# patflick/psac

Hardware: AMD Instinct MI355X
Metric: MChars/s SA+LCP build; rank-pair radix-sort HBM GB/s vs peak (higher is better)
Workload: dtype u64

## Files before the change

### include/psacx.h

```cpp
#ifndef PSACX_H
#define PSACX_H

#include <stddef.h>
#include <stdint.h>

#ifdef __cplusplus
extern "C" {
#endif

typedef struct psacx_ctx psacx_ctx;

enum {
    PSACX_OK = 0,
    PSACX_EINVAL = -1,
    PSACX_ERANGE = -2,
    PSACX_ENOMEM = -3,
    PSACX_EHIP = -4,
    PSACX_EDEVICE = -5,
    PSACX_ENOGPU = -6
};

enum {
    PSACX_LCP = 1u,
    PSACX_NO_FAST = 2u,
// ... 13 lines not shown

typedef struct psacx_stats {
    uint32_t sigma;
    uint32_t bits_per_char;
    uint32_t k;
    uint32_t n_rounds;
    psacx_round rounds[PSACX_MAX_ROUNDS];
    double ms_total;
    double ms_alphabet, ms_kmer, ms_sort_hist, ms_sort_scatter, ms_rebucket, ms_isa_scatter,
           ms_gather, ms_compact, ms_rmq_build, ms_finalize;
    double ms_sort_scatter3, ms_sort_tilehist, ms_sort_scatter2;
    uint64_t scatter_launches[3];
    uint64_t scatter_records[3];
    uint64_t scatter_bytes[3];
    uint64_t hist_bytes;
    uint64_t workspace_bytes;
    uint64_t onew_passes;
    uint64_t heavy_rounds;
    uint64_t heavy_records;
    uint64_t light_records;
    uint64_t level_gathers;
    double ms_host[9];
    uint64_t locate_fetches[2];
} psacx_stats;


#define PSACX_STREAM_DEFAULT ((void*)(intptr_t)-1)
int psacx_create(psacx_ctx** out, int device, void* stream);
void psacx_destroy(psacx_ctx* ctx);
const char* psacx_strerror(int code);
const char* psacx_last_hip_error(const psacx_ctx* ctx);
int psacx_trim(psacx_ctx* ctx);

enum {
    PSACX_OPT_RESET = 0, PSACX_OPT_FORCE_DIET, PSACX_OPT_DIET_CAP, PSACX_OPT_ONE_STAGE, PSACX_OPT_TIES_RADIX, PSACX_OPT_NO_ONE_WORD,
    PSACX_OPT_ONE_WORD_ALWAYS, PSACX_OPT_ONE_WORD_MIN, PSACX_OPT_WIDEN_LAST, PSACX_OPT_NO_DIGIT_BYTES, PSACX_OPT_NO_BUCKET_SORT,
    PSACX_OPT_ISA_UPDATE, PSACX_OPT_GATHER, PSACX_OPT_NO_HEAVY, PSACX_OPT_NO_WHOLE, PSACX_OPT_NO_LAZY_RANKS, PSACX_OPT_NO_EARLY_OUT,
    PSACX_OPT_NO_SPREAD_CURSORS, PSACX_OPT_LOCATE_SHAPE, PSACX_OPT_LOCATE_COUNT, PSACX_OPT_COUNT
};
int psacx_configure(psacx_ctx* ctx, int option, uint64_t value);
int psacx_configure_from_env(psacx_ctx* ctx);
const char* psacx_debug_env(const char* name);

int psacx_construct_u32(psacx_ctx* ctx, const uint8_t* text, uint64_t n, uint32_t k,
                        uint32_t flags, uint32_t* SA, uint32_t* ISA, uint32_t* LCP);
int psacx_construct_u64(psacx_ctx* ctx, const uint8_t* text, uint64_t n, uint32_t k,
                        uint32_t flags, uint64_t* SA, uint64_t* ISA, uint64_t* LCP);
int psacx_construct_dev_u32(psacx_ctx* ctx, const uint8_t* d_text, uint64_t n, uint32_t k,
                            uint32_t flags, uint32_t* d_SA, uint32_t* d_ISA, uint32_t* d_LCP);
int psacx_construct_dev_u64(psacx_ctx* ctx, const uint8_t* d_text, uint64_t n, uint32_t k,
                            uint32_t flags, uint64_t* d_SA, uint64_t* d_ISA, uint64_t* d_LCP);

int psacx_construct_lc_u32(psacx_ctx* ctx, const uint8_t* text, uint64_t n, uint32_t k, uint32_t flags,
                           uint32_t* SA, uint32_t* ISA, uint32_t* LCP, uint8_t* Lc);
int psacx_construct_lc_u64(psacx_ctx* ctx, const uint8_t* text, uint64_t n, uint32_t k, uint32_t flags,
                           uint64_t* SA, uint64_t* ISA, uint64_t* LCP, uint8_t* Lc);
int psacx_construct_lc_dev_u32(psacx_ctx* ctx, const uint8_t* d_text, uint64_t n, uint32_t k, uint32_t flags,
                               uint32_t* d_SA, uint32_t* d_ISA, uint32_t* d_LCP, uint8_t* d_Lc);
int psacx_construct_lc_dev_u64(psacx_ctx* ctx, const uint8_t* d_text, uint64_t n, uint32_t k, uint32_t flags,
                               uint64_t* d_SA, uint64_t* d_ISA, uint64_t* d_LCP, uint8_t* d_Lc);

// ... 178 lines not shown
```

### psac_amd/_lib.py

```python
import ctypes as C
import os

_HERE = os.path.dirname(os.path.abspath(__file__))
LIB_PATH = os.path.join(_HERE, "lib", "libpsacx.so")

PSACX_LCP = 1
PSACX_NO_FAST = 2
PSACX_PROFILE = 4
PSACX_MAX_ROUNDS = 72

OPTIONS = {"reset": 0, "force_diet": 1, "diet_cap": 2, "one_stage": 3, "ties_radix": 4, "no_one_word": 5, "one_word_always": 6, "one_word_min": 7,
           "widen_last": 8, "no_digit_bytes": 9, "no_bucket_sort": 10, "isa_update": 11, "gather": 12, "no_heavy": 13, "no_whole": 14, "no_lazy_ranks": 15, "no_early_out": 16,
           "no_spread_cursors": 17, "locate_shape": 18, "locate_count": 19}
MULTI_OPTIONS = {"layout": 1, "slab": 2, "output_slack": 3, "trace": 4, "wire_piece": 5, "pieces": 6, "check_chunks": 7, "global_refine_sort": 8,
                 "one_stage": 9, "two_word": 10, "one_word": 11, "no_slices": 12, "slice_wide": 13, "slice_shape": 14}
MULTI_FORCE_WIRE, MULTI_NO_RCCL, MULTI_SHM = 1, 2, 4
ENV_KNOBS = bool(os.environ.get("PSACX_ENV_KNOBS"))
if ENV_KNOBS and os.environ.get("PSACX_LIB"):
    LIB_PATH = os.environ["PSACX_LIB"]

EXPORTS = [
    "psacx_create", "psacx_destroy", "psacx_strerror", "psacx_last_hip_error", "psacx_trim", "psacx_configure", "psacx_configure_from_env", "psacx_debug_env",
    "psacx_construct_u32", "psacx_construct_u64", "psacx_construct_dev_u32", "psacx_construct_dev_u64",
    "psacx_construct_gsa_u32", "psacx_construct_gsa_u64", "psacx_construct_gsa_dev_u32", "psacx_construct_gsa_dev_u64",
    "psacx_construct_lc_u32", "psacx_construct_lc_u64", "psacx_construct_lc_dev_u32", "psacx_construct_lc_dev_u64",
    "psacx_get_stats", "psacx_profile", "psacx_check_dev_u32", "psacx_check_dev_u64", "psacx_check_gsa_dev_u32", "psacx_check_gsa_dev_u64", "psacx_pair_sort_dev_u32", "psacx_pair_sort_dev_u64", "psacx_ansv_u32",
    "psacx_ansv_u64", "psacx_ansv_dev_u32", "psacx_ansv_dev_u64", "psacx_suffix_tree_u32", "psacx_suffix_tree_u64", "psacx_suffix_tree_dev_u32", "psacx_suffix_tree_dev_u64",
    "psacx_check_suffix_tree_dev_u32", "psacx_check_suffix_tree_dev_u64",
    "psacx_suffix_tree_gsa_u32", "psacx_suffix_tree_gsa_u64", "psacx_suffix_tree_gsa_dev_u32", "psacx_suffix_tree_gsa_dev_u64",
    "psacx_check_suffix_tree_gsa_dev_u32", "psacx_check_suffix_tree_gsa_dev_u64", "psacx_dev_alloc", "psacx_dev_free", "psacx_copy_h2d", "psacx_copy_d2h", "psacx_sync",
    "psacx_rand_dna", "psacx_synth_text_dev",
    "psacx_lookup_table_dev_u32", "psacx_lookup_table_dev_u64", "psacx_locate_dev_u32", "psacx_locate_dev_u64", "psacx_locate_u32", "psacx_locate_u64",
    "psacx_multi_create", "psacx_multi_unique_id", "psacx_multi_create_rank", "psacx_multi_destroy", "psacx_multi_nranks",
    "psacx_multi_nlocal", "psacx_multi_uses_rccl", "psacx_multi_last_error", "psacx_multi_ctx", "psacx_multi_construct_dev_u32",
    "psacx_multi_construct_dev_u64", "psacx_multi_construct_u32", "psacx_multi_construct_u64", "psacx_multi_get_stats",
    "psacx_multi_check_dev_u32", "psacx_multi_check_dev_u64", "psacx_multi_check_gsa_dev_u32", "psacx_multi_check_gsa_dev_u64", "psacx_multi_ansv_dev_u32", "psacx_multi_ansv_dev_u64",
# ... 1 lines not shown
    "psacx_multi_suffix_tree_dev_u32", "psacx_multi_suffix_tree_dev_u64", "psacx_multi_suffix_tree_u32", "psacx_multi_suffix_tree_u64",
    "psacx_multi_left_chars_dev_u32", "psacx_multi_left_chars_dev_u64", "psacx_multi_construct_lc_u32", "psacx_multi_construct_lc_u64",
    "psacx_multi_configure", "psacx_multi_configure_from_env", "psacx_multi_create_ex", "psacx_multi_create_rank_ex", "psacx_multi_get_memory", "psacx_multi_transport", "psacx_multi_get_wire", "psacx_multi_get_phases", "psacx_multi_last_form",
]


class Round(C.Structure):
    _fields_ = [("h", C.c_uint64), ("active", C.c_uint64), ("unfinished_buckets", C.c_uint64),
                ("unfinished_elements", C.c_uint64), ("sort_passes", C.c_uint32),
                ("sort_passes_skipped", C.c_uint32)]


class Stats(C.Structure):
    _fields_ = [("sigma", C.c_uint32), ("bits_per_char", C.c_uint32), ("k", C.c_uint32),
                ("n_rounds", C.c_uint32), ("rounds", Round * PSACX_MAX_ROUNDS),
                ("ms_total", C.c_double), ("ms_alphabet", C.c_double), ("ms_kmer", C.c_double),
                ("ms_sort_hist", C.c_double), ("ms_sort_scatter", C.c_double), ("ms_rebucket", C.c_double),
                ("ms_isa_scatter", C.c_double), ("ms_gather", C.c_double), ("ms_compact", C.c_double),
                ("ms_rmq_build", C.c_double), ("ms_finalize", C.c_double),
                ("ms_sort_scatter3", C.c_double), ("ms_sort_tilehist", C.c_double), ("ms_sort_scatter2", C.c_double),
                ("scatter_launches", C.c_uint64 * 3), ("scatter_records", C.c_uint64 * 3),
                ("scatter_bytes", C.c_uint64 * 3), ("hist_bytes", C.c_uint64), ("workspace_bytes", C.c_uint64), ("onew_passes", C.c_uint64),
                ("heavy_rounds", C.c_uint64), ("heavy_records", C.c_uint64), ("light_records", C.c_uint64), ("level_gathers", C.c_uint64),
                ("ms_host", C.c_double * 9), ("locate_fetches", C.c_uint64 * 2)]


class PsacxError(RuntimeError):
    def __init__(self, code, msg):
        RuntimeError.__init__(self, "psacx error %d: %s" % (code, msg))
        self.code = code


_lib = None


def load():
    global _lib
    if _lib is not None:
        return _lib
    if not os.path.exists(LIB_PATH):
        raise ImportError("libpsacx.so not built (%s); run `python -c 'import __graft_entry__ as g; g.build()'`"
                          % LIB_PATH)
    try:
        import torch
    except ImportError:
        pass
    lib = C.CDLL(LIB_PATH, mode=C.RTLD_GLOBAL)
# ... 111 lines not shown
```

### psac_amd/csrc/construct.hpp

```cpp
#pragma once
#include <chrono>
#include <thread>
#include "engine.hpp"
#include "bucket_sort.hpp"
#include "heavy_keys.hpp"

namespace psacx {

constexpr int SCAN_ITEMS = 8;
#ifndef RB1W_BLOCK
#define RB1W_BLOCK 512
#endif
template <typename T> struct ScanCfg {
    static constexpr int BLOCK = sizeof(T) == 8 ? 512 : 768;
    static constexpr int TILE = BLOCK * SCAN_ITEMS;
};
constexpr int SCAN_TILE_MIN = 512 * SCAN_ITEMS;

constexpr unsigned SCAN_CHUNKS = 4096, SCAN_CHUNK = 1024 * 4;
template <typename T> struct Work {
    T *bsa;
    SortBufs<T> x, y;
    SortBufs<T> ry;
    T *pos_a, *pos_b;
// ... 291 lines not shown
        kin = o.k1; vin = o.k2;
    }
    const uint64_t nwin = (n + (1ull << INV_WINDOW_BITS) - 1) >> INV_WINDOW_BITS;
    hipLaunchKernelGGL((window_scatter_kernel<T, T, 512>), dim3((unsigned)nwin), dim3(512), 0, c->stream, kin, vin, n, d_isa);
    PSACX_HIP(c, hipGetLastError());
    return PSACX_OK;
}

template <typename T> struct IsaLevels {
    static constexpr int PB = 512, PI = 16, WB = ISA_NARROW_WB, CB = ISA_NARROW_CB;
    psacx_ctx* c; unsigned* cursors; uint64_t n; int lv9; uint64_t* lvl_a; bool open; unsigned stripes;
    unsigned* c0() const { return cursors; }
    unsigned* c1() const { return cursors + 1024; }
    int begin(psacx_ctx* ctx, unsigned* d_cursors, uint64_t n_, uint64_t* a, const Knobs& kn) {
        c = ctx; cursors = d_cursors; n = n_; lvl_a = a; open = true;
        lv9 = isa_narrow_levels<T>(n, kn);
        stripes = isa_stripes(kn);
        if (lv9 < 1 || lv9 > 2) { c->hip_err = "ISA update by levels: text size out of range"; return PSACX_EINVAL; }
        PSACX_HIP(c, hipMemsetAsync(cursors, 0, (1024 + (size_t)(n >> WB) + 1) * sizeof(unsigned), c->stream));
        return PSACX_OK;
    }
    int add(const uint64_t* pairs, uint64_t cnt, const ulonglong2* skip = nullptr) {
        static_assert((PB * PI) % ScanCfg<T>::TILE == 0 || sizeof(T) != 8, "a tile of pairs covers whole scan tiles");
        hipLaunchKernelGGL((partition_packed_kernel<T, PB, PI, 0, CB>), dim3(striped_grid((cnt + PB * PI - 1) / (PB * PI), stripes)), dim3(PB), 0, c->stream, (const T*)nullptr,
                           (const T*)nullptr, pairs, lvl_a, cnt, isa_narrow_shift(lv9, 0), lv9 == 1 ? c1() : c0(), (uint64_t)0, (const unsigned*)nullptr, 0u,
                           (const uint32_t*)nullptr, (uint64_t)0, (uint64_t)0, skip, skip ? (unsigned)((PB * PI) / ScanCfg<T>::TILE) : 0u, stripes);
        PSACX_HIP(c, hipGetLastError());
        return PSACX_OK;
    }
    int finish(T* d_isa, uint64_t* lvl_b) {
        open = false;
        const uint64_t* last = lvl_a;
        if (lv9 == 2) {
            hipLaunchKernelGGL((partition_packed_kernel<T, PB, PI, 0, CB>), dim3(striped_grid((n + PB * PI - 1) / (PB * PI), stripes)), dim3(PB), 0, c->stream, (const T*)nullptr,
                               (const T*)nullptr, (const uint64_t*)lvl_a, lvl_b, n, (unsigned)WB, c1(), (uint64_t)0, (const unsigned*)c0(), isa_narrow_shift(lv9, 0),
                               (const uint32_t*)nullptr, (uint64_t)0, (uint64_t)0, (const ulonglong2*)nullptr, 0u, stripes);
            PSACX_HIP(c, hipGetLastError());
            last = lvl_b;
        }
        hipLaunchKernelGGL((window_store_sparse_kernel<T, 1024, WB>), dim3((unsigned)((n + (1ull << WB) - 1) >> WB)), dim3(1024), 0, c->stream, last, (const unsigned*)c1(), n, d_isa);
        PSACX_HIP(c, hipGetLastError());
        return PSACX_OK;
    }
};

template <typename T>
// ... 383 lines not shown
        T* const pyr1 = (WITH_LCP && w.pyr.nlev > 1) ? w.pyr.lvl[1] : (T*)nullptr;
        isa_hist_ready = !fuse32 && isa_radix_levels<T>(n, kn) && (uint64_t)ScanCfg<T>::TILE == (uint64_t)ScatterCfg<T>::TILE;
        unsigned* const sa_hist = isa_hist_ready ? reinterpret_cast<unsigned*>(w.sc.d_desc + 256) : (unsigned*)nullptr;
        if (gsa) {
            PSACX_TRY((run_carries<T, false, true>(c, w, sorted.k1, sorted.k2, nullptr, n, d_sa, ks)));
            hipLaunchKernelGGL((rebucket_first_kernel<T, ScanCfg<T>::BLOCK, SCAN_ITEMS, WITH_LCP, true>), dim3((unsigned)ntiles),
                               dim3(ScanCfg<T>::BLOCK), 0, c->stream, sorted.k1, sorted.k2, d_sa, n, ks, w.bsa, d_lcp,
                               w.d_carry, w.d_nact, w.d_nunf, n, Boundary<T>(), pyr1, sa_hist, (int)INV_WINDOW_BITS);
        } else if (fuse32) {
            PSACX_TRY((run_carries<T, false>(c, w, sorted.k1, sorted.k2, nullptr, n, d_sa, ks)));
            PSACX_HIP(c, hipMemsetAsync(w.d_cursors, 0, ((size_t)1 << ISA_NARROW_CB) * sizeof(unsigned) + sizeof(unsigned), c->stream));
            launch_rebucket_first_fused<T, WITH_LCP>(c, (unsigned)ntiles, sorted.k1, sorted.k2, d_sa, n, ks, w.bsa, d_lcp, w.d_carry, w.d_nact,
                                                     w.d_nunf, pyr1, reinterpret_cast<uint32_t*>(w.x.v), reinterpret_cast<uint32_t*>(w.y.v),
                                                     isa_narrow_shift(isa_levels32(n), 0), w.d_cursors);
        } else if (fuse_l1 && onew_recs) {
            if constexpr (sizeof(T) == 8) {
                hipLaunchKernelGGL(last_head_1w_kernel<0>, dim3((unsigned)((ntiles + 3) / 4)), dim3(256), 0, c->stream, reinterpret_cast<const uint64_t*>(sorted.k1),
                                   reinterpret_cast<const uint64_t*>(onew_w1), reinterpret_cast<const uint64_t*>(sorted.k2), n, (unsigned)ScanCfg<T>::TILE, ntiles,
                                   w.d_carry, ks, onew_view);
                PSACX_HIP(c, hipGetLastError());
                PSACX_TRY(scan_carries<T>(c, w, ntiles));
                PSACX_HIP(c, hipMemsetAsync(w.d_cursors, 0, ((size_t)1 << ISA_NARROW_CB) * sizeof(unsigned) + sizeof(unsigned), c->stream));
                lazy_ids = n >= (1ull << 22);
                hipLaunchKernelGGL((rebucket_first_kernel<T, RB1W_BLOCK, ScanCfg<T>::TILE / RB1W_BLOCK, WITH_LCP, false, ISA_NARROW_CB, true, true>), dim3((unsigned)ntiles),
                                   dim3(RB1W_BLOCK), 0, c->stream, sorted.k1, sorted.k2, (const T*)nullptr, n, ks, w.bsa, d_lcp, w.d_carry, w.d_nact, w.d_nunf, n,
                                   Boundary<T>(), pyr1, (unsigned*)nullptr, 0, reinterpret_cast<uint32_t*>(w.x.v), (uint32_t*)nullptr,
                                   isa_narrow_shift(isa_narrow_levels<T>(n, kn), 0), w.d_cursors, d_sa, lazy_ids ? 1 : 0, onew_view, (const T*)onew_w1);
            }
        } else if (fuse_l1) {
            PSACX_TRY((run_carries<T, false>(c, w, sorted.k1, sorted.k2, nullptr, n, d_sa, ks)));
            PSACX_HIP(c, hipMemsetAsync(w.d_cursors, 0, ((size_t)1 << ISA_NARROW_CB) * sizeof(unsigned) + sizeof(unsigned), c->stream));
            uint32_t* const pk = reinterpret_cast<uint32_t*>(w.x.v);
            lazy_ids = n >= (1ull << 22);
            launch_rebucket_first_fused<T, WITH_LCP>(c, (unsigned)ntiles, sorted.k1, sorted.k2, d_sa, n, ks, w.bsa, d_lcp, w.d_carry, w.d_nact,
                                                     w.d_nunf, pyr1, pk, (uint32_t*)nullptr,
                                                     isa_narrow_shift(isa_narrow_levels<T>(n, kn), 0), w.d_cursors, lazy_ids ? 1 : 0);
        } else {
            PSACX_TRY((run_carries<T, false>(c, w, sorted.k1, sorted.k2, nullptr, n, d_sa, ks)));
            hipLaunchKernelGGL((rebucket_first_kernel<T, ScanCfg<T>::BLOCK, SCAN_ITEMS, WITH_LCP>), dim3((unsigned)ntiles),
                               dim3(ScanCfg<T>::BLOCK), 0, c->stream, sorted.k1, sorted.k2, d_sa, n, ks, w.bsa, d_lcp,
                               w.d_carry, w.d_nact, w.d_nunf, n, Boundary<T>(), pyr1, sa_hist, (int)INV_WINDOW_BITS);
        }
        PSACX_HIP(c, hipGetLastError());
    }
    if (c->first_round_hook && !gsa && c->early_word) {
        const uint64_t ntiles = (n + ScanCfg<T>::TILE - 1) / ScanCfg<T>::TILE;
// ... 531 lines not shown
```

### psac_amd/csrc/engine.hpp

```cpp
#pragma once
#include <hip/hip_runtime.h>

#include <algorithm>
#include <cstdio>
#include <cstdlib>
#include <cstring>
#include <condition_variable>
#include <functional>
#include <map>
#include <mutex>
#include <string>
#include <thread>
#include <sched.h>
#include <pthread.h>
#include <cctype>
#include <cstdio>
#include <vector>

#include "../../include/psacx.h"
#include "radix.hpp"
#include "sa_kernels.hpp"

namespace psacx {

// ... 5 lines not shown
}

namespace psacx { struct HostPool; }

namespace psacx {
struct Knobs {
    bool force_diet = false;
    uint64_t diet_cap = 0;
    bool one_stage = false;
    bool ties_radix = false;
    bool no_one_word = false;
    bool one_word_always = false;
    unsigned one_word_min = 24;
    int isa_update = 0;
    bool no_digit_bytes = false;
    bool no_bucket_sort = false;
    int gather = 0;
    bool no_heavy = false;
    bool no_early_out = false;
    bool no_lazy_ranks = false;
    bool no_whole = false;
    bool widen_last = false;
    bool no_spread_cursors = false;
    int locate_shape = 0;
    bool locate_count = false;
};

}

struct psacx_ctx {
    int device = 0;
    hipStream_t stream = nullptr;
    bool own_stream = false;
    char* slab = nullptr;
    size_t slab_bytes = 0;
    char* aux = nullptr;
    size_t aux_bytes = 0;
    char* pinned = nullptr;
    char* pinned_dev = nullptr;
    size_t pinned_bytes = 0;
    char* io = nullptr;
    size_t io_bytes = 0;
    static constexpr int STAGE_SLOTS = 4;
    char* stage[STAGE_SLOTS] = {nullptr, nullptr, nullptr, nullptr};
    char* dstage = nullptr;
    size_t stage_bytes = 0;
// ... 957 lines not shown
```

### psac_amd/csrc/heavy_keys.hpp

```cpp
#pragma once
#include "sa_kernels.hpp"

namespace psacx {

constexpr unsigned HEAVY_MAXB = 4096;
constexpr unsigned HEAVY_PAD = 1;

struct HeavyTabs {
    uint64_t* bstart;
    uint64_t* value;
    unsigned long long* eq;
    unsigned long long* less;
    unsigned long long* light;
    uint64_t* lstart;
    uint64_t* rank;
    static size_t words(unsigned nb) { return (size_t)(nb + 1) * 2 + (size_t)nb * (HEAVY_PAD + 3) + 8; }
};
constexpr uint64_t HEAVY_KEEP = 1ull << 63;

__device__ __forceinline__ uint64_t heavy_lower_bound(const uint32_t* __restrict__ ord, uint64_t cnt, uint32_t b) {
    uint64_t lo = 0, hi = cnt;
    while (lo < hi) { const uint64_t m = lo + ((hi - lo) >> 1); if (ord[m] < b) lo = m + 1; else hi = m; }
    return lo;
}

template <typename T>
__global__ void heavy_probe_kernel(const uint32_t* __restrict__ ord, uint64_t cnt, uint32_t nb, const T* __restrict__ pos, const T* __restrict__ SA,
                                   const T* __restrict__ ISA, uint64_t n, uint64_t h, HeavyTabs ht) {
    const uint32_t b = blockIdx.x * blockDim.x + threadIdx.x;
// ... 117 lines not shown
```

### psac_amd/csrc/psacx_abi.hip

```cpp
#include "engine.hpp"

namespace psacx {
int construct_dev_u32(psacx_ctx*, const uint8_t*, uint64_t, uint32_t, uint32_t, uint32_t*, uint32_t*, uint32_t*);
int construct_dev_u64(psacx_ctx*, const uint8_t*, uint64_t, uint32_t, uint32_t, uint64_t*, uint64_t*, uint64_t*);
int construct_host_u32(psacx_ctx*, const uint8_t*, uint64_t, uint32_t, uint32_t, uint32_t*, uint32_t*, uint32_t*);
int construct_gsa_host_u32(psacx_ctx*, const uint8_t*, uint64_t, const uint64_t*, uint64_t, uint32_t, uint32_t, uint32_t*, uint32_t*, uint32_t*);
int construct_gsa_dev_u32(psacx_ctx*, const uint8_t*, uint64_t, const uint64_t*, uint64_t, uint32_t, uint32_t, uint32_t*, uint32_t*, uint32_t*);
int construct_gsa_host_u64(psacx_ctx*, const uint8_t*, uint64_t, const uint64_t*, uint64_t, uint32_t, uint32_t, uint64_t*, uint64_t*, uint64_t*);
int construct_gsa_dev_u64(psacx_ctx*, const uint8_t*, uint64_t, const uint64_t*, uint64_t, uint32_t, uint32_t, uint64_t*, uint64_t*, uint64_t*);
int construct_lc_host_u32(psacx_ctx*, const uint8_t*, uint64_t, uint32_t, uint32_t, uint32_t*, uint32_t*, uint32_t*, uint8_t*);
int construct_lc_host_u64(psacx_ctx*, const uint8_t*, uint64_t, uint32_t, uint32_t, uint64_t*, uint64_t*, uint64_t*, uint8_t*);
int construct_lc_dev_u32(psacx_ctx*, const uint8_t*, uint64_t, uint32_t, uint32_t, uint32_t*, uint32_t*, uint32_t*, uint8_t*);
int construct_lc_dev_u64(psacx_ctx*, const uint8_t*, uint64_t, uint32_t, uint32_t, uint64_t*, uint64_t*, uint64_t*, uint8_t*);
int construct_host_u64(psacx_ctx*, const uint8_t*, uint64_t, uint32_t, uint32_t, uint64_t*, uint64_t*, uint64_t*);
int pair_sort_dev_u32(psacx_ctx*, uint32_t*, uint32_t*, uint32_t*, uint64_t, uint32_t);
int pair_sort_dev_u64(psacx_ctx*, uint64_t*, uint64_t*, uint64_t*, uint64_t, uint32_t);
int check_dev_u32(psacx_ctx*, const uint8_t*, uint64_t, const uint32_t*, const uint32_t*, const uint32_t*, uint64_t*);
int check_dev_u64(psacx_ctx*, const uint8_t*, uint64_t, const uint64_t*, const uint64_t*, const uint64_t*, uint64_t*);
int check_gsa_dev_u32(psacx_ctx*, const uint8_t*, uint64_t, const uint64_t*, uint64_t, const uint32_t*, const uint32_t*, const uint32_t*, uint64_t*);
int check_gsa_dev_u64(psacx_ctx*, const uint8_t*, uint64_t, const uint64_t*, uint64_t, const uint64_t*, const uint64_t*, const uint64_t*, uint64_t*);
int synth_text_dev(psacx_ctx*, uint8_t*, uint64_t, uint64_t, int, uint64_t, uint64_t);
int suffix_tree_host_u32(psacx_ctx*, const uint8_t*, uint64_t, const uint32_t*, const uint32_t*, uint64_t*, uint32_t*);
int suffix_tree_host_u64(psacx_ctx*, const uint8_t*, uint64_t, const uint64_t*, const uint64_t*, uint64_t*, uint32_t*);
int suffix_tree_dev_u32(psacx_ctx*, const uint8_t*, uint64_t, const uint32_t*, const uint32_t*, uint64_t*, uint32_t*, uint64_t*);
// ... 83 lines not shown
    if (!c) return PSACX_EINVAL;
    psacx::Knobs& k = c->knobs;
    switch (option) {
    case PSACX_OPT_RESET: k = psacx::Knobs(); return PSACX_OK;
    case PSACX_OPT_FORCE_DIET: k.force_diet = value != 0; return PSACX_OK;
    case PSACX_OPT_DIET_CAP: k.diet_cap = value; return PSACX_OK;
    case PSACX_OPT_ONE_STAGE: k.one_stage = value != 0; return PSACX_OK;
    case PSACX_OPT_TIES_RADIX: k.ties_radix = value != 0; return PSACX_OK;
    case PSACX_OPT_NO_ONE_WORD: k.no_one_word = value != 0; return PSACX_OK;
    case PSACX_OPT_ONE_WORD_ALWAYS: k.one_word_always = value != 0; return PSACX_OK;
    case PSACX_OPT_ONE_WORD_MIN: if (value > 62) return PSACX_EINVAL; k.one_word_min = value ? (unsigned)std::max<uint64_t>(16, value) : 24u; return PSACX_OK;
    case PSACX_OPT_WIDEN_LAST: k.widen_last = value != 0; return PSACX_OK;
    case PSACX_OPT_NO_DIGIT_BYTES: k.no_digit_bytes = value != 0; return PSACX_OK;
    case PSACX_OPT_NO_BUCKET_SORT: k.no_bucket_sort = value != 0; return PSACX_OK;
    case PSACX_OPT_ISA_UPDATE: if (value > 2) return PSACX_EINVAL; k.isa_update = (int)value; return PSACX_OK;
    case PSACX_OPT_GATHER: if (value > 2) return PSACX_EINVAL; k.gather = (int)value; return PSACX_OK;
    case PSACX_OPT_NO_HEAVY: k.no_heavy = value != 0; return PSACX_OK;
    case PSACX_OPT_NO_WHOLE: k.no_whole = value != 0; return PSACX_OK;
    case PSACX_OPT_NO_LAZY_RANKS: k.no_lazy_ranks = value != 0; return PSACX_OK;
    case PSACX_OPT_NO_EARLY_OUT: k.no_early_out = value != 0; return PSACX_OK;
    case PSACX_OPT_NO_SPREAD_CURSORS: k.no_spread_cursors = value != 0; return PSACX_OK;
    case PSACX_OPT_LOCATE_SHAPE: if (value > 2) return PSACX_EINVAL; k.locate_shape = (int)value; return PSACX_OK;
    case PSACX_OPT_LOCATE_COUNT: k.locate_count = value != 0; return PSACX_OK;
    default: return PSACX_EINVAL;
    }
}

const char* psacx_debug_env(const char* name) { return name ? getenv(name) : nullptr; }

int psacx_configure_from_env(psacx_ctx* c) {
    if (!c) return PSACX_EINVAL;
    static const struct { const char* name; int option; } flags[] = {
        {"PSACX_FORCE_DIET", PSACX_OPT_FORCE_DIET}, {"PSACX_ONE_STAGE", PSACX_OPT_ONE_STAGE}, {"PSACX_TIES_RADIX", PSACX_OPT_TIES_RADIX},
        {"PSACX_NO_ONE_WORD", PSACX_OPT_NO_ONE_WORD}, {"PSACX_ONE_WORD_ALWAYS", PSACX_OPT_ONE_WORD_ALWAYS}, {"PSACX_WIDEN_LAST", PSACX_OPT_WIDEN_LAST},
        {"PSACX_NO_DIGIT_BYTES", PSACX_OPT_NO_DIGIT_BYTES}, {"PSACX_NO_BUCKET_SORT", PSACX_OPT_NO_BUCKET_SORT}, {"PSACX_NO_HEAVY", PSACX_OPT_NO_HEAVY},
        {"PSACX_NO_WHOLE", PSACX_OPT_NO_WHOLE}, {"PSACX_NO_LAZY_RANKS", PSACX_OPT_NO_LAZY_RANKS},
        {"PSACX_NO_EARLY_OUT", PSACX_OPT_NO_EARLY_OUT}, {"PSACX_NO_SPREAD_CURSORS", PSACX_OPT_NO_SPREAD_CURSORS},
        {"PSACX_LOCATE_COUNT", PSACX_OPT_LOCATE_COUNT}};
    (void)psacx_configure(c, PSACX_OPT_RESET, 0);
    for (const auto& f : flags) if (psacx_debug_env(f.name)) (void)psacx_configure(c, f.option, 1);
    if (const char* e = psacx_debug_env("PSACX_DIET_CAP")) (void)psacx_configure(c, PSACX_OPT_DIET_CAP, strtoull(e, nullptr, 10));
    if (const char* e = psacx_debug_env("PSACX_ONE_WORD_MIN")) (void)psacx_configure(c, PSACX_OPT_ONE_WORD_MIN, strtoull(e, nullptr, 10));
    if (const char* e = psacx_debug_env("PSACX_ISA_UPDATE")) (void)psacx_configure(c, PSACX_OPT_ISA_UPDATE, e[0] == 's' ? 1 : 2);
    if (const char* e = psacx_debug_env("PSACX_LOCATE_SHAPE")) (void)psacx_configure(c, PSACX_OPT_LOCATE_SHAPE, e[0] == 'g' ? 2 : 1);
    if (const char* e = psacx_debug_env("PSACX_GATHER")) (void)psacx_configure(c, PSACX_OPT_GATHER, e[0] == 'f' ? 1 : 2);
    return PSACX_OK;
}

int psacx_trim(psacx_ctx* c) {
    if (!c) return PSACX_EINVAL;
    PSACX_HIP(c, hipSetDevice(c->device));
    PSACX_HIP(c, hipStreamSynchronize(c->stream));
    if (c->slab) { PSACX_HIP(c, hipFree(c->slab)); c->slab = nullptr; c->slab_bytes = 0; }
    if (c->aux) { PSACX_HIP(c, hipFree(c->aux)); c->aux = nullptr; c->aux_bytes = 0; }
    if (c->io) { PSACX_HIP(c, hipFree(c->io)); c->io = nullptr; c->io_bytes = 0; }
    if (c->dstage) { PSACX_HIP(c, hipFree(c->dstage)); c->dstage = nullptr; }
    for (int i = 0; i < psacx_ctx::STAGE_SLOTS; ++i) {
        if (c->stage[i]) { (void)hipHostFree(c->stage[i]); c->stage[i] = nullptr; }
        if (c->stage_ev[i]) { (void)hipEventDestroy(c->stage_ev[i]); c->stage_ev[i] = nullptr; }
    }
    delete c->hpool; c->hpool = nullptr;
// ... 167 lines not shown
```

### psac_amd/csrc/sa_kernels.hpp

```cpp
#pragma once
#ifndef RB_WAVES_ATTR
#define RB_WAVES_ATTR
#endif
#ifndef RB_ABLATE
#define RB_ABLATE 0
#endif
#include <type_traits>
#include "dev_common.hpp"

namespace psacx {

constexpr int RADIX_P = 256;

struct CodeTable { uint16_t c[256]; };

template <typename T>
__device__ __forceinline__ void key_summary_add(unsigned long long* partials, T or1, T and1, T or2, T and2) {
    __shared__ unsigned long long red[4][16];
    or1 = wave_reduce<T>(or1, OpOr()); and1 = wave_reduce<T>(and1, OpAnd());
    or2 = wave_reduce<T>(or2, OpOr()); and2 = wave_reduce<T>(and2, OpAnd());
    const unsigned wave = threadIdx.x / WAVE, nw = (blockDim.x + WAVE - 1) / WAVE;
    const unsigned long long hi = ~(unsigned long long)(T)~(T)0;
    if (lane_id() == 0) {
        red[0][wave] = (unsigned long long)or1; red[1][wave] = (unsigned long long)and1 | hi;
        red[2][wave] = (unsigned long long)or2; red[3][wave] = (unsigned long long)and2 | hi;
    }
    __syncthreads();
    if (threadIdx.x < 4) {
        unsigned long long v = red[threadIdx.x][0];
        for (unsigned w = 1; w < nw; ++w) v = (threadIdx.x & 1) ? (v & red[threadIdx.x][w]) : (v | red[threadIdx.x][w]);
        partials[(size_t)blockIdx.x * 4 + threadIdx.x] = v;
// ... 897 lines not shown
#pragma unroll
            for (int j = 0; j < ITEMS; ++j) {
                const unsigned p = tid + j * BLOCK;
                if (p < count) {
                    const uint32_t x = (uint32_t)stage[p];
                    dest[j] = pbase[(x >> part_shift) & (NCLS - 1)] + p;
                    part_key[dest[j]] = x;
                }
            }
            __syncthreads();
#pragma unroll
            for (int j = 0; j < ITEMS; ++j)
                if (e0 + j < n) stage[slot[j]] = (uint32_t)(id[j] - 1);
            __syncthreads();
#pragma unroll
            for (int j = 0; j < ITEMS; ++j) {
                const unsigned p = tid + j * BLOCK;
                if (p < count) part_val[dest[j]] = (uint32_t)stage[p];
            }
        }
    }
}

template <typename T>
__global__ void isa_scatter_kernel(const T* __restrict__ SA, const T* __restrict__ Bsa, uint64_t n,
                                   T* __restrict__ ISA, uint64_t koff) {
    const uint64_t stride = (uint64_t)gridDim.x * blockDim.x;
    for (uint64_t i = (uint64_t)blockIdx.x * blockDim.x + threadIdx.x; i < n; i += stride)
        ISA[(uint64_t)SA[i] - koff] = Bsa[i] - 1;
}

constexpr int INV_WINDOW_BITS = 12;

template <typename TI, typename TO, int BLOCK, int ITEMS, bool SUB1 = false, int CB = 8>
__global__ __launch_bounds__(BLOCK) void partition_pairs_kernel(
    const TI* __restrict__ key_in, const TI* __restrict__ val_in, TO* __restrict__ key_out,
    TO* __restrict__ val_out, uint64_t n, unsigned shift, unsigned* __restrict__ cursors, uint64_t koff) {
    constexpr int NCLS = 1 << CB;
    static_assert(BLOCK >= NCLS, "one thread per class");
    constexpr int TILE = BLOCK * ITEMS;
    __shared__ TO stage[TILE];
    __shared__ unsigned cnt[NCLS];
    __shared__ unsigned bstart[NCLS];
    __shared__ uint64_t gbase[NCLS];
    __shared__ unsigned scan_tmp[BLOCK / WAVE + 1];
    const unsigned tid = threadIdx.x;
// ... 1155 lines not shown
```

Before: 25670.

## Add specialized one-word first rebucket kernel with fused partition for u64

Adds a specialized first-round rebucket kernel for the one-word key layout. It computes head flags and LCP bytes from packed rank/SA words, bucket boundaries and tie windows, then writes Bsa, LCP, SA and the partitioned rank pairs in one pass. It is enabled by default when the shape fits, with a config flag to fall back to the generic kernel. The aim is to cut memory traffic and instruction cost in the first rebucket step. The price is a large block of special-case code whose correctness depends on packed-field assumptions.

```diff
diff --git a/include/psacx.h b/include/psacx.h
--- a/include/psacx.h
+++ b/include/psacx.h
@@ -59,6 +59,7 @@
     uint64_t level_gathers;
     double ms_host[9];
     uint64_t locate_fetches[2];
+    uint64_t rebucket_1w;
 } psacx_stats;
 
 
@@ -73,7 +74,8 @@
     PSACX_OPT_RESET = 0, PSACX_OPT_FORCE_DIET, PSACX_OPT_DIET_CAP, PSACX_OPT_ONE_STAGE, PSACX_OPT_TIES_RADIX, PSACX_OPT_NO_ONE_WORD,
     PSACX_OPT_ONE_WORD_ALWAYS, PSACX_OPT_ONE_WORD_MIN, PSACX_OPT_WIDEN_LAST, PSACX_OPT_NO_DIGIT_BYTES, PSACX_OPT_NO_BUCKET_SORT,
     PSACX_OPT_ISA_UPDATE, PSACX_OPT_GATHER, PSACX_OPT_NO_HEAVY, PSACX_OPT_NO_WHOLE, PSACX_OPT_NO_LAZY_RANKS, PSACX_OPT_NO_EARLY_OUT,
-    PSACX_OPT_NO_SPREAD_CURSORS, PSACX_OPT_LOCATE_SHAPE, PSACX_OPT_LOCATE_COUNT, PSACX_OPT_COUNT
+    PSACX_OPT_NO_SPREAD_CURSORS, PSACX_OPT_LOCATE_SHAPE, PSACX_OPT_LOCATE_COUNT, PSACX_OPT_GENERIC_REBUCKET,
+    PSACX_OPT_COUNT
 };
 int psacx_configure(psacx_ctx* ctx, int option, uint64_t value);
 int psacx_configure_from_env(psacx_ctx* ctx);
diff --git a/psac_amd/_lib.py b/psac_amd/_lib.py
--- a/psac_amd/_lib.py
+++ b/psac_amd/_lib.py
@@ -11,7 +11,7 @@
 
 OPTIONS = {"reset": 0, "force_diet": 1, "diet_cap": 2, "one_stage": 3, "ties_radix": 4, "no_one_word": 5, "one_word_always": 6, "one_word_min": 7,
            "widen_last": 8, "no_digit_bytes": 9, "no_bucket_sort": 10, "isa_update": 11, "gather": 12, "no_heavy": 13, "no_whole": 14, "no_lazy_ranks": 15, "no_early_out": 16,
-           "no_spread_cursors": 17, "locate_shape": 18, "locate_count": 19}
+           "no_spread_cursors": 17, "locate_shape": 18, "locate_count": 19, "generic_rebucket": 20}
 MULTI_OPTIONS = {"layout": 1, "slab": 2, "output_slack": 3, "trace": 4, "wire_piece": 5, "pieces": 6, "check_chunks": 7, "global_refine_sort": 8,
                  "one_stage": 9, "two_word": 10, "one_word": 11, "no_slices": 12, "slice_wide": 13, "slice_shape": 14}
 MULTI_FORCE_WIRE, MULTI_NO_RCCL, MULTI_SHM = 1, 2, 4
@@ -59,7 +59,7 @@
                 ("scatter_launches", C.c_uint64 * 3), ("scatter_records", C.c_uint64 * 3),
                 ("scatter_bytes", C.c_uint64 * 3), ("hist_bytes", C.c_uint64), ("workspace_bytes", C.c_uint64), ("onew_passes", C.c_uint64),
                 ("heavy_rounds", C.c_uint64), ("heavy_records", C.c_uint64), ("light_records", C.c_uint64), ("level_gathers", C.c_uint64),
-                ("ms_host", C.c_double * 9), ("locate_fetches", C.c_uint64 * 2)]
+                ("ms_host", C.c_double * 9), ("locate_fetches", C.c_uint64 * 2), ("rebucket_1w", C.c_uint64)]
 
 
 class PsacxError(RuntimeError):
diff --git a/psac_amd/csrc/construct.hpp b/psac_amd/csrc/construct.hpp
--- a/psac_amd/csrc/construct.hpp
+++ b/psac_amd/csrc/construct.hpp
@@ -337,6 +337,7 @@
     }
     int add(const uint64_t* pairs, uint64_t cnt, const ulonglong2* skip = nullptr) {
         static_assert((PB * PI) % ScanCfg<T>::TILE == 0 || sizeof(T) != 8, "a tile of pairs covers whole scan tiles");
+        static_assert((PB * PI) / ScanCfg<T>::TILE == 2 || sizeof(T) != 8, "rebucket_pure_kernel finds the other scan tile of a tile of pairs as tile ^ 1");
         hipLaunchKernelGGL((partition_packed_kernel<T, PB, PI, 0, CB>), dim3(striped_grid((cnt + PB * PI - 1) / (PB * PI), stripes)), dim3(PB), 0, c->stream, (const T*)nullptr,
                            (const T*)nullptr, pairs, lvl_a, cnt, isa_narrow_shift(lv9, 0), lv9 == 1 ? c1() : c0(), (uint64_t)0, (const unsigned*)nullptr, 0u,
                            (const uint32_t*)nullptr, (uint64_t)0, (uint64_t)0, skip, skip ? (unsigned)((PB * PI) / ScanCfg<T>::TILE) : 0u, stripes);
@@ -766,6 +767,15 @@
                 PSACX_TRY(scan_carries<T>(c, w, ntiles));
                 PSACX_HIP(c, hipMemsetAsync(w.d_cursors, 0, ((size_t)1 << ISA_NARROW_CB) * sizeof(unsigned) + sizeof(unsigned), c->stream));
                 lazy_ids = n >= (1ull << 22);
+                if (!kn.generic_rebucket && rb1w_fits(ks.lc, ks.c1, ks.c2, onew_view.low, onew_view.sfield, n)) {
+                    c->stats.rebucket_1w = 1;
+                    hipLaunchKernelGGL((rebucket_first_1w_kernel<RB1W_BLOCK, ScanCfg<T>::TILE / RB1W_BLOCK, WITH_LCP, ISA_NARROW_CB>), dim3((unsigned)ntiles), dim3(RB1W_BLOCK), 0,
+                                       c->stream, reinterpret_cast<const uint64_t*>(sorted.k1), reinterpret_cast<const uint64_t*>(onew_w1),
+                                       reinterpret_cast<const uint64_t*>(sorted.k2), n, onew_view, rb1w_shape(ks.lc, ks.c1, ks.c2, onew_view.low, onew_view.sfield, n),
+                                       reinterpret_cast<uint64_t*>(w.bsa), reinterpret_cast<uint64_t*>(d_lcp), w.d_carry, w.d_nact, w.d_nunf,
+                                       reinterpret_cast<uint64_t*>(pyr1), reinterpret_cast<uint64_t*>(w.x.v),
+                                       isa_narrow_shift(isa_narrow_levels<T>(n, kn), 0), w.d_cursors, reinterpret_cast<uint64_t*>(d_sa), lazy_ids ? 1 : 0);
+                } else
                 hipLaunchKernelGGL((rebucket_first_kernel<T, RB1W_BLOCK, ScanCfg<T>::TILE / RB1W_BLOCK, WITH_LCP, false, ISA_NARROW_CB, true, true>), dim3((unsigned)ntiles),
                                    dim3(RB1W_BLOCK), 0, c->stream, sorted.k1, sorted.k2, (const T*)nullptr, n, ks, w.bsa, d_lcp, w.d_carry, w.d_nact, w.d_nunf, n,
                                    Boundary<T>(), pyr1, (unsigned*)nullptr, 0, reinterpret_cast<uint32_t*>(w.x.v), (uint32_t*)nullptr,
diff --git a/psac_amd/csrc/engine.hpp b/psac_amd/csrc/engine.hpp
--- a/psac_amd/csrc/engine.hpp
+++ b/psac_amd/csrc/engine.hpp
@@ -51,6 +51,7 @@
     bool no_whole = false;
     bool widen_last = false;
     bool no_spread_cursors = false;
+    bool generic_rebucket = false;
     int locate_shape = 0;
     bool locate_count = false;
 };
diff --git a/psac_amd/csrc/heavy_keys.hpp b/psac_amd/csrc/heavy_keys.hpp
--- a/psac_amd/csrc/heavy_keys.hpp
+++ b/psac_amd/csrc/heavy_keys.hpp
@@ -5,6 +5,7 @@
 
 constexpr unsigned HEAVY_MAXB = 4096;
 constexpr unsigned HEAVY_PAD = 1;
+static_assert(HEAVY_PAD == 1, "HeavyView (sa_kernels.hpp) reads the counters as eq[b]");
 
 struct HeavyTabs {
     uint64_t* bstart;
diff --git a/psac_amd/csrc/psacx_abi.hip b/psac_amd/csrc/psacx_abi.hip
--- a/psac_amd/csrc/psacx_abi.hip
+++ b/psac_amd/csrc/psacx_abi.hip
@@ -129,6 +129,7 @@
     case PSACX_OPT_NO_SPREAD_CURSORS: k.no_spread_cursors = value != 0; return PSACX_OK;
     case PSACX_OPT_LOCATE_SHAPE: if (value > 2) return PSACX_EINVAL; k.locate_shape = (int)value; return PSACX_OK;
     case PSACX_OPT_LOCATE_COUNT: k.locate_count = value != 0; return PSACX_OK;
+    case PSACX_OPT_GENERIC_REBUCKET: k.generic_rebucket = value != 0; return PSACX_OK;
     default: return PSACX_EINVAL;
     }
 }
@@ -143,7 +144,7 @@
         {"PSACX_NO_DIGIT_BYTES", PSACX_OPT_NO_DIGIT_BYTES}, {"PSACX_NO_BUCKET_SORT", PSACX_OPT_NO_BUCKET_SORT}, {"PSACX_NO_HEAVY", PSACX_OPT_NO_HEAVY},
         {"PSACX_NO_WHOLE", PSACX_OPT_NO_WHOLE}, {"PSACX_NO_LAZY_RANKS", PSACX_OPT_NO_LAZY_RANKS},
         {"PSACX_NO_EARLY_OUT", PSACX_OPT_NO_EARLY_OUT}, {"PSACX_NO_SPREAD_CURSORS", PSACX_OPT_NO_SPREAD_CURSORS},
-        {"PSACX_LOCATE_COUNT", PSACX_OPT_LOCATE_COUNT}};
+        {"PSACX_LOCATE_COUNT", PSACX_OPT_LOCATE_COUNT}, {"PSACX_GENERIC_REBUCKET", PSACX_OPT_GENERIC_REBUCKET}};
     (void)psacx_configure(c, PSACX_OPT_RESET, 0);
     for (const auto& f : flags) if (psacx_debug_env(f.name)) (void)psacx_configure(c, f.option, 1);
     if (const char* e = psacx_debug_env("PSACX_DIET_CAP")) (void)psacx_configure(c, PSACX_OPT_DIET_CAP, strtoull(e, nullptr, 10));
diff --git a/psac_amd/csrc/rebucket_1w_math.hpp b/psac_amd/csrc/rebucket_1w_math.hpp
--- /dev/null
+++ b/psac_amd/csrc/rebucket_1w_math.hpp
@@ -0,0 +1,68 @@
+#pragma once
+#include <cstdint>
+
+#if defined(__HIPCC__)
+#define RB1W_HD __host__ __device__ __forceinline__
+#else
+#define RB1W_HD inline
+#endif
+
+namespace psacx {
+
+constexpr unsigned RB1W_DIGIT_BITS = 8;
+constexpr unsigned RB1W_RECIP_SHIFT = 10;
+
+RB1W_HD unsigned rb1w_clz32(uint32_t x) { return x ? (unsigned)__builtin_clz(x) : 32u; }
+RB1W_HD unsigned rb1w_clz64(uint64_t x) { return x ? (unsigned)__builtin_clzll(x) : 64u; }
+
+RB1W_HD uint32_t rb1w_recip(unsigned lc) { return ((1u << RB1W_RECIP_SHIFT) + lc - 1u) / lc; }
+RB1W_HD unsigned rb1w_chars(unsigned bits, uint32_t recip) { return (bits * recip) >> RB1W_RECIP_SHIFT; }
+
+struct Rb1wShape {
+    uint32_t recip;
+    uint32_t low;
+    uint32_t sfield;
+    uint32_t two_k;
+    uint32_t nm1;
+    uint32_t bits1, bits2;
+    uint32_t c1;
+};
+inline Rb1wShape rb1w_shape(unsigned lc, unsigned c1, unsigned c2, unsigned low, unsigned sfield, uint64_t n) {
+    Rb1wShape s;
+    s.recip = rb1w_recip(lc); s.low = low; s.sfield = sfield; s.two_k = c1 + c2; s.nm1 = (uint32_t)(n - 1);
+    s.bits1 = c1 * lc; s.bits2 = c2 * lc; s.c1 = c1;
+    return s;
+}
+inline bool rb1w_fits(unsigned lc, unsigned c1, unsigned c2, unsigned low, unsigned sfield, uint64_t n) {
+    return n >= 1 && n <= (1ull << 32) && lc >= 1 && lc <= 8 && c1 + c2 <= 255 && low <= 32 && sfield >= 32 && low + sfield == 64 && c1 * lc <= 64 && c2 * lc <= 64 &&
+           RB1W_DIGIT_BITS + low <= c1 * lc;
+}
+
+RB1W_HD unsigned rb1w_lead_lcp_rest(uint32_t ra, uint32_t rb, const Rb1wShape& s) {
+    return rb1w_chars(RB1W_DIGIT_BITS + s.low - 32u + rb1w_clz32(ra ^ rb), s.recip);
+}
+RB1W_HD unsigned rb1w_lead_lcp_bucket(unsigned ba, unsigned bb, const Rb1wShape& s) {
+    return rb1w_chars(rb1w_clz32((uint32_t)(ba ^ bb)) - (32u - RB1W_DIGIT_BITS), s.recip);
+}
+RB1W_HD unsigned rb1w_lead_lcp(unsigned ba, uint32_t ra, unsigned bb, uint32_t rb, const Rb1wShape& s) {
+    if (ba != bb) return rb1w_lead_lcp_bucket(ba, bb, s);
+    if (ra != rb) return rb1w_lead_lcp_rest(ra, rb, s);
+    return s.two_k;
+}
+RB1W_HD unsigned rb1w_window_lcp(uint64_t x1, uint64_t x2, uint64_t y1, uint64_t y2, const Rb1wShape& s) {
+    if (x1 != y1) return rb1w_chars(rb1w_clz64(x1 ^ y1) - (64u - s.bits1), s.recip);
+    if (x2 != y2) return s.c1 + rb1w_chars(rb1w_clz64(x2 ^ y2) - (64u - s.bits2), s.recip);
+    return s.two_k;
+}
+
+RB1W_HD bool rb1w_short(uint32_t sa, const Rb1wShape& s) { return s.nm1 - sa < s.two_k - 1u; }
+RB1W_HD unsigned rb1w_cap(unsigned c, uint32_t sa, const Rb1wShape& s) {
+    const uint32_t rem = s.nm1 - sa;
+    return (rb1w_short(sa, s) && rem + 1u < c) ? rem + 1u : c;
+}
+
+RB1W_HD uint32_t rb1w_rank_of_head(uint64_t e) { return (uint32_t)e; }
+RB1W_HD uint32_t rb1w_rank_of_id(uint64_t id) { return (uint32_t)(id - 1u); }
+RB1W_HD uint64_t rb1w_id_of_rank(uint32_t rank) { return (uint64_t)rank + 1u; }
+
+}
diff --git a/psac_amd/csrc/sa_kernels.hpp b/psac_amd/csrc/sa_kernels.hpp
--- a/psac_amd/csrc/sa_kernels.hpp
+++ b/psac_amd/csrc/sa_kernels.hpp
@@ -7,6 +7,7 @@
 #endif
 #include <type_traits>
 #include "dev_common.hpp"
+#include "rebucket_1w_math.hpp"
 
 namespace psacx {
 
@@ -950,6 +951,261 @@
     }
 }
 
+template <typename F>
+__device__ __forceinline__ void rb1w_store_run(uint64_t* __restrict__ p, uint64_t wb, uint64_t n, unsigned lane, uint64_t* xw, F f) {
+    constexpr int ITEMS = 8, ROW = WAVE + WAVE / 8;
+    uint64_t* const run = xw + lane * (ITEMS + 1);
+#pragma unroll
+    for (int j = 0; j < ITEMS; ++j) run[j] = f(j);
+    xrun_order();
+    const uint64_t* const rows = xw + lane + (lane >> 3);
+    uint64_t r[ITEMS];
+#pragma unroll
+    for (int i = 0; i < ITEMS; ++i) r[i] = rows[i * ROW];
+    xrun_order();
+    uint64_t* __restrict__ q = p + wb + lane;
+    if (wb + (uint64_t)WAVE * ITEMS <= n) {
+#pragma unroll
+        for (int i = 0; i < ITEMS; ++i) q[i * WAVE] = r[i];
+    } else {
+#pragma unroll
+        for (int i = 0; i < ITEMS; ++i) if (wb + (uint64_t)i * WAVE + lane < n) q[i * WAVE] = r[i];
+    }
+}
+__device__ __forceinline__ unsigned rb1w_fresh(unsigned x) { asm volatile("" : "+v"(x)); return x; }
+__device__ __forceinline__ unsigned rb1w_fresh_uniform(unsigned x) { asm volatile("" : "+s"(x)); return x; }
+
+template <int BLOCK, int ITEMS, bool WITH_LCP, int PCB = 9>
+__global__ __launch_bounds__(BLOCK, 6) void rebucket_first_1w_kernel(
+    const uint64_t* __restrict__ S1, const uint64_t* __restrict__ S1t, const uint64_t* __restrict__ S2, uint64_t n, OneWordView ow, Rb1wShape sh,
+    uint64_t* __restrict__ Bsa, uint64_t* __restrict__ LCP, const uint64_t* __restrict__ carry_in, uint64_t* __restrict__ n_active,
+    uint64_t* __restrict__ n_unf, uint64_t* __restrict__ pyr1, uint64_t* __restrict__ part_out, unsigned part_shift,
+    unsigned* __restrict__ part_cursors, uint64_t* __restrict__ sa_out, int lazy_ids) {
+    constexpr int TILE = BLOCK * ITEMS, NW = BLOCK / WAVE, NCLS = 1 << PCB;
+    static_assert(ITEMS == 8, "eight LCP bytes in two words, eight head flags and the next one in a mask");
+    static_assert(BLOCK >= 257 && BLOCK >= NCLS, "one thread per table entry and per class");
+    static_assert(TILE < (1 << 16), "both counters of a tile reduced in one word");
+    static_assert(64 % ITEMS == 0, "a group of 64 entries must sit inside one wave");
+    constexpr size_t XP_RUNS = sizeof(uint64_t) * NW * XRUN_WORDS<ITEMS>::N, XP_STAGE = sizeof(uint64_t) * (size_t)TILE;
+    __shared__ __attribute__((aligned(16))) unsigned char xp_raw[XP_RUNS > XP_STAGE ? XP_RUNS : XP_STAGE];
+    __shared__ unsigned long long s_off[257];
+    __shared__ uint32_t s_last[NW][2];
+    __shared__ unsigned s_scan[NW], s_h0[NW], s_cnt[NW];
+    __shared__ unsigned pcnt[NCLS], pstart[NCLS], pscan_tmp[NW + 1];
+    __shared__ uint64_t pbase[NCLS];
+    const unsigned tid = threadIdx.x, lane = lane_id(), wave = tid / WAVE;
+    const unsigned tile = blockIdx.x;
+    const uint64_t tbase = (uint64_t)tile * TILE;
+    const uint64_t e0 = tbase + (uint64_t)tid * ITEMS;
+    uint64_t* const xw = reinterpret_cast<uint64_t*>(xp_raw) + wave * XRUN_WORDS<ITEMS>::N;
+    const unsigned nv = e0 + ITEMS <= n ? (unsigned)ITEMS : (e0 < n ? (unsigned)(n - e0) : 0u);
+    const unsigned vmask = (1u << nv) - 1u;
+    const bool have_p = e0 > 0;
+
+    const unsigned long long my_off = tid < 257 ? ow.off[tid] : 0ull;
+    const uint64_t carry64 = carry_in[tile];
+    uint64_t xprev = 0, xnext = 0;
+    if (tid == 0 && have_p) xprev = S1[e0 - 1];
+    const bool have_tq = tid == BLOCK - 1 && e0 + ITEMS < n;
+    if (have_tq) xnext = S1[e0 + ITEMS];
+    uint32_t rest[ITEMS], sa[ITEMS];
+    {
+        uint64_t x[ITEMS];
+        load_run_x<uint64_t, ITEMS>(S1, e0, n, x, 0ull, xw);
+#pragma unroll
+        for (int j = 0; j < ITEMS; ++j) { rest[j] = (uint32_t)(x[j] >> sh.sfield); sa[j] = (uint32_t)x[j]; }
+    }
+    for (int i = tid; i < NCLS; i += BLOCK) pcnt[i] = 0;
+    if (tid < 257) s_off[tid] = my_off;
+    if (lane == WAVE - 1) { s_last[wave][0] = rest[ITEMS - 1]; s_last[wave][1] = sa[ITEMS - 1]; }
+    __syncthreads();
+    ow.off = s_off;
+    uint32_t prest = (uint32_t)__shfl_up((int)rest[ITEMS - 1], 1, WAVE), psa = (uint32_t)__shfl_up((int)sa[ITEMS - 1], 1, WAVE);
+    if (lane == 0) {
+        if (wave) { prest = s_last[wave - 1][0]; psa = s_last[wave - 1][1]; }
+        else { prest = (uint32_t)(xprev >> sh.sfield); psa = (uint32_t)xprev; }
+    }
+
+    uint32_t lcb[2] = {0u, 0u};
+    {
+        uint32_t pr = prest;
+#pragma unroll
+        for (int j = 0; j < ITEMS; ++j) { lcb[j >> 2] |= rb1w_lead_lcp_rest(pr, rest[j], sh) << ((j & 3) * 8); pr = rest[j]; }
+    }
+    unsigned bdiff = 0;
+    if (nv) {
+        OneWordCursor cu;
+        cu.start(ow, have_p ? e0 - 1 : 0);
+        if (cu.end <= e0 + nv) {
+            unsigned pb = cu.b;
+#pragma unroll
+            for (int j = 0; j <= ITEMS; ++j) {
+                if (e0 + j < n) {
+                    const unsigned b = cu.at(ow, e0 + j);
+                    if (b != pb) {
+                        bdiff |= 1u << j;
+                        if (j < ITEMS) lcb[(j & 7) >> 2] = (lcb[(j & 7) >> 2] & ~(0xFFu << ((j & 3) * 8))) | (rb1w_lead_lcp_bucket(pb, b, sh) << ((j & 3) * 8));
+                    }
+                    pb = b;
+                }
+            }
+        }
+    }
+    unsigned eqp = 0;
+    {
+        uint32_t pr = prest;
+#pragma unroll
+        for (int j = 0; j < ITEMS; ++j) {
+            if (rest[j] == pr && !((bdiff >> j) & 1u) && (j || have_p)) eqp |= 1u << j;
+            pr = rest[j];
+        }
+        eqp &= vmask;
+    }
+    if (eqp) {
+        const unsigned tied = eqp | (eqp >> 1);
+        uint64_t p1 = 0, p2 = 0;
+        if (eqp & 1u) { p1 = S1t[e0 - 1]; p2 = S2[e0 - 1]; }
+#pragma unroll
+        for (int h = 0; h < ITEMS; h += 4) {
+            uint64_t t1[4], t2[4];
+#pragma unroll
+            for (int j = 0; j < 4; ++j) {
+                const bool t = (tied >> (h + j)) & 1u;
+                t1[j] = t ? S1t[e0 + h + j] : 0ull; t2[j] = t ? S2[e0 + h + j] : 0ull;
+            }
+#pragma unroll
+            for (int j = 0; j < 4; ++j) {
+                if ((eqp >> (h + j)) & 1u) {
+                    const unsigned c = rb1w_window_lcp(p1, p2, t1[j], t2[j], sh);
+                    lcb[h >> 2] = (lcb[h >> 2] & ~(0xFFu << (j * 8))) | (c << (j * 8));
+                }
+                p1 = t1[j]; p2 = t2[j];
+            }
+        }
+    }
+    unsigned heads = 0;
+    {
+        uint32_t ps = psa;
+#pragma unroll
+        for (int j = 0; j < ITEMS; ++j) {
+            unsigned c = (lcb[j >> 2] >> ((j & 3) * 8)) & 0xFFu;
+            c = rb1w_cap(rb1w_cap(c, ps, sh), sa[j], sh);
+            const bool very_first = j == 0 && !have_p;
+            if (very_first) c = 0;
+            if (very_first || c < sh.two_k || !((vmask >> j) & 1u)) heads |= 1u << j;
+            lcb[j >> 2] = (lcb[j >> 2] & ~(0xFFu << ((j & 3) * 8))) | (c << ((j & 3) * 8));
+            ps = sa[j];
+        }
+    }
+    bool tile_next_head = true;
+    if (have_tq) {
+        const uint32_t qrest = (uint32_t)(xnext >> sh.sfield), qsa = (uint32_t)xnext;
+        if (qrest == rest[ITEMS - 1] && !((bdiff >> ITEMS) & 1u)) {
+            const uint64_t e = e0 + ITEMS;
+            unsigned c = rb1w_window_lcp(S1t[e - 1], S2[e - 1], S1t[e], S2[e], sh);
+            c = rb1w_cap(rb1w_cap(c, sa[ITEMS - 1], sh), qsa, sh);
+            tile_next_head = c < sh.two_k;
+        }
+    }
+    const unsigned hm = heads & vmask;
+    const unsigned run = hm ? tid * ITEMS + (32u - (unsigned)__builtin_clz(hm)) : 0u;
+    const unsigned inc = wave_scan_inclusive<unsigned>(run, OpMax());
+    if (lane == WAVE - 1) s_scan[wave] = inc;
+    if (lane == 0) s_h0[wave] = heads & 1u;
+    __syncthreads();
+    unsigned excl = 0;
+#pragma unroll
+    for (int w = 0; w < NW; ++w) { const unsigned s = s_scan[w]; if ((unsigned)w < wave && s > excl) excl = s; }
+    {
+        const unsigned prev = (unsigned)__shfl_up((int)inc, 1, WAVE);
+        if (lane && prev > excl) excl = prev;
+        unsigned nh = (unsigned)__shfl_down((int)(heads & 1u), 1, WAVE);
+        if (lane == WAVE - 1) nh = wave + 1 < NW ? s_h0[wave + 1] : (tile_next_head ? 1u : 0u);
+        heads |= nh << ITEMS;
+    }
+    unsigned nact = 0, nub = 0;
+#pragma unroll
+    for (int j = 0; j < ITEMS; ++j) {
+        if ((vmask >> j) & 1u) {
+            const bool h = (heads >> j) & 1u, hn = (heads >> (j + 1)) & 1u;
+            if (!h || !hn) ++nact;
+            if (h && !hn) ++nub;
+        }
+    }
+    {
+        const unsigned both = wave_reduce<unsigned>(nact | (nub << 16), OpSum());
+        if (lane == 0) s_cnt[wave] = both;
+    }
+    uint32_t slot2[ITEMS / 2];
+#pragma unroll
+    for (int j = 0; j < ITEMS; ++j) {
+        const unsigned d = (sa[j] >> part_shift) & (NCLS - 1);
+        const unsigned sl = (vmask >> j) & 1u ? atomicAdd(&pcnt[d], 1u) : 0u;
+        slot2[j >> 1] = (j & 1) ? (slot2[j >> 1] | (sl << 16)) : sl;
+    }
+    __syncthreads();
+    unsigned both_counts = 0;
+#pragma unroll
+    for (int w = 0; w < NW; ++w) both_counts += s_cnt[w];
+    const unsigned tact = both_counts & 0xFFFFu, tub = both_counts >> 16;
+    if (tid == 0) { n_active[tile] = tact; n_unf[tile] = tub; }
+    const uint32_t carry0 = excl ? (uint32_t)tbase + excl - 1u : rb1w_rank_of_id(carry64);
+    const uint64_t wb = e0 - (uint64_t)lane * ITEMS;
+    if (!(lazy_ids && tact == 0)) {
+        const unsigned hf = rb1w_fresh(hm);
+        rb1w_store_run(Bsa, wb, n, lane, xw, [&](int j) {
+            const unsigned m = hf & ((2u << j) - 1u);
+            return rb1w_id_of_rank(m ? rb1w_rank_of_head(e0) + (31u - (unsigned)__builtin_clz(m)) : carry0);
+        });
+    }
+    if (WITH_LCP)
+        rb1w_store_run(LCP, wb, n, lane, xw, [&](int j) { return (heads >> j) & 1u ? (uint64_t)((lcb[j >> 2] >> ((j & 3) * 8)) & 0xFFu) : n; });
+    rb1w_store_run(sa_out, wb, n, lane, xw, [&](int j) { return (uint64_t)sa[j]; });
+    if (WITH_LCP && pyr1) {
+        uint32_t m = ~0u;
+#pragma unroll
+        for (int j = 0; j < ITEMS; ++j) {
+            const uint32_t c = (lcb[j >> 2] >> ((j & 3) * 8)) & 0xFFu;
+            if ((hm >> j) & 1u && c < m) m = c;
+        }
+#pragma unroll
+        for (int d = 1; d < 64 / ITEMS; d <<= 1) { const uint32_t o = shfl_xor<uint32_t>(m, d); m = o < m ? o : m; }
+        if ((tid & (64 / ITEMS - 1)) == 0 && e0 < n) pyr1[e0 >> 6] = m == ~0u ? n : (uint64_t)m;
+    }
+    uint64_t* const stage = reinterpret_cast<uint64_t*>(xp_raw);
+    const unsigned count = n - tbase < (uint64_t)TILE ? (unsigned)(n - tbase) : (unsigned)TILE;
+    const unsigned tot = tid < NCLS ? pcnt[tid] : 0u;
+    unsigned total;
+    const unsigned bs = block_scan_exclusive<BLOCK, unsigned>(tot, OpSum(), 0u, pscan_tmp, &total);
+    if (tid < NCLS) {
+        pstart[tid] = bs;
+        if (tot) {
+            const unsigned at = atomicAdd(&part_cursors[tid], tot);
+            pbase[tid] = ((uint64_t)tid << part_shift) + at - bs;
+        }
+    }
+    __syncthreads();
+    {
+        const unsigned hf = rb1w_fresh(hm), shift2 = rb1w_fresh_uniform(part_shift);
+#pragma unroll
+        for (int j = 0; j < ITEMS; ++j) {
+            const unsigned d = (sa[j] >> shift2) & (NCLS - 1);
+            const unsigned m = hf & ((2u << j) - 1u);
+            const uint32_t rank = m ? rb1w_rank_of_head(e0) + (31u - (unsigned)__builtin_clz(m)) : carry0;
+            if ((vmask >> j) & 1u) stage[((slot2[j >> 1] >> ((j & 1) * 16)) & 0xFFFFu) + pstart[d]] = (uint64_t)sa[j] | ((uint64_t)rank << 32);
+        }
+    }
+    __syncthreads();
+#pragma unroll
+    for (int j = 0; j < ITEMS; ++j) {
+        const unsigned p = tid + j * BLOCK;
+        if (p < count) {
+            const uint64_t x = stage[p];
+            part_out[pbase[((uint32_t)x >> part_shift) & (NCLS - 1)] + p] = x;
+        }
+    }
+}
+
 template <typename T>
 __global__ void isa_scatter_kernel(const T* __restrict__ SA, const T* __restrict__ Bsa, uint64_t n,
                                    T* __restrict__ ISA, uint64_t koff) {
```

After: 26100, median of 6. 1.7% higher.
